# FrontierDevelopmentLab/2024-HL-SPI3S-SuNeRF

Hardware: AMD Instinct MI355X
Metric: ray-samples/sec (fwd+bwd, fused emission renderer) (higher is better)
Workload: dtype f32 (forward: every operand split into an fp16 head and an exact remainder, head products on the fp16 matrix cores + block-scaled fp8 products for the two cross terms; backward: fp16 MFMA, W^T as a single fp16 image (measured policy); fp32 accumulate and parameters)

## Files before the change

### 2024-hl-spi3s-sunerf_amd/csrc/bwd_pipe.hip

```cpp
#include "grad_common.h"
#include <mutex>
#include <vector>

namespace {

constexpr int PD = 256, PKS = PD / 16, PNT = PD / 32, PT = 8;
constexpr int WG = 512;
constexpr int WG_PRE = 256;
constexpr int NBUF = 4;
constexpr int NBUF_H = 5;
#ifndef PIPE_DMA_ON_WEIGHT
#define PIPE_DMA_ON_WEIGHT 2
#endif
#ifndef PIPE_ZD
#define PIPE_ZD 2
#endif
#ifndef PIPE_RING
#define PIPE_RING 16
#endif
#ifndef PIPE_POLL_LAG
#define PIPE_POLL_LAG 2
#endif
constexpr int RING = PIPE_RING;
constexpr int SLOT = PKS * 1024;
#ifndef PIPE_LDS_IMAGE
#define PIPE_LDS_IMAGE 1
#endif
static_assert(PIPE_LDS_IMAGE >= 0 && PIPE_LDS_IMAGE <= 2, "PIPE_LDS_IMAGE: 0, 1 or 2");
constexpr int FRAG_H = PIPE_LDS_IMAGE ? 1088 : 1024;
constexpr int BUF_HID = 24 * FRAG_H;
constexpr int BUF_IN = 16 * 1024;
constexpr int BUF_PRE = 19 * 1024;
constexpr unsigned SPIN_LIMIT = 50000000u;

constexpr unsigned ST_OK = 0, ST_START_TIMEOUT = 1, ST_PLACEMENT = 2, ST_WAIT_TIMEOUT = 3;

struct PipeArgs {
  const char* packedT;
  const char* act_stash;
  const char* dz_top;
  char* rings;
  unsigned* ctrl;
  float* partial;
  const float* g_raw;
  const unsigned* g_absmax_bits;
  float* partial_out;
  int64_t n_chunks_total;
  int S, n_chunks;
  int n_linear, d_out;
  int NP, NPX;
  int hi_only;
  int inject;
  unsigned* dbg;
};

__host__ __device__ inline size_t ctrl_counter_word(int n_links, int P, int link, int which) {
  return 64 + (((size_t)P * n_links + link) * 4 + which) * 32;
}
__host__ __device__ inline size_t ctrl_bytes(int NP, int n_links) { return (64 + (size_t)NP * n_links * 4 * 32) * 4; }

typedef __attribute__((address_space(1))) unsigned gu32;
__device__ __forceinline__ unsigned ld_agent(const unsigned* p) {
  return __hip_atomic_load((const gu32*)p, __ATOMIC_RELAXED, __HIP_MEMORY_SCOPE_AGENT);
}
__device__ __forceinline__ void st_agent(unsigned* p, unsigned v) {
  __hip_atomic_store((gu32*)p, v, __ATOMIC_RELAXED, __HIP_MEMORY_SCOPE_AGENT);
}

template <int POLICY>
__device__ __forceinline__ void dma_piece(const char* src_lane, unsigned lds_dst) {
  const unsigned d = __builtin_amdgcn_readfirstlane(lds_dst);
  if (POLICY == 1) asm volatile("s_mov_b32 m0, %1\n\ts_nop 0\n\tglobal_load_lds_dwordx4 %0, off nt" :: "v"(src_lane), "s"(d) : "memory");
  else if (POLICY == 2) asm volatile("s_mov_b32 m0, %1\n\ts_nop 0\n\tglobal_load_lds_dwordx4 %0, off sc1" :: "v"(src_lane), "s"(d) : "memory");
  else asm volatile("s_mov_b32 m0, %1\n\ts_nop 0\n\tglobal_load_lds_dwordx4 %0, off" :: "v"(src_lane), "s"(d) : "memory");
}
template <int POLICY>
__device__ __forceinline__ void dma_piece_s(const char* src_uniform, unsigned voff, unsigned lds_dst) {
  const unsigned d = __builtin_amdgcn_readfirstlane(lds_dst);
#ifndef PIPE_STREAM_BITS
#define PIPE_STREAM_BITS "nt"
#endif
  if (POLICY == 1) asm volatile("s_mov_b32 m0, %1\n\ts_nop 0\n\tglobal_load_lds_dwordx4 %0, %2 " PIPE_STREAM_BITS :: "v"(voff), "s"(d), "s"(src_uniform) : "memory");
  else if (POLICY == 2) asm volatile("s_mov_b32 m0, %1\n\ts_nop 0\n\tglobal_load_lds_dwordx4 %0, %2 sc1" :: "v"(voff), "s"(d), "s"(src_uniform) : "memory");
  else asm volatile("s_mov_b32 m0, %1\n\ts_nop 0\n\tglobal_load_lds_dwordx4 %0, %2" :: "v"(voff), "s"(d), "s"(src_uniform) : "memory");
}
__device__ __forceinline__ void dma_poll(const unsigned* src_lane, unsigned lds_dst) {
  const unsigned d = __builtin_amdgcn_readfirstlane(lds_dst);
  asm volatile("s_mov_b32 m0, %1\n\ts_nop 0\n\tglobal_load_lds_dword %0, off sc1" :: "v"(src_lane), "s"(d) : "memory");
}

__device__ __forceinline__ void store_tile(const f32x16& t, float* dst) {
  const Rsrc r = make_rsrc(dst, 16 * 64 * 4);
  const int lo4 = (int)(threadIdx.x & 63u) * 4;
#pragma unroll
  for (int g = 0; g < 16; ++g) {
    const float te = t[g];
    unsigned tv;
    asm volatile("v_accvgpr_read_b32 %0, %1" : "=v"(tv) : "a"(te));
    __builtin_amdgcn_raw_buffer_store_b32(tv, r, lo4, g * 256, 0);
    if ((g & 3) == 3) __builtin_amdgcn_sched_barrier(0);
  }
}

__device__ __forceinline__ void mfma_agpr(f32x16& acc, const half8& a, const half8& b) {
  asm volatile("v_mfma_f32_32x32x16_f16 %0, %1, %2, %0" : "+a"(acc) : "v"(a), "v"(b));
}
__device__ __forceinline__ void drain_matrix_pipe() { asm volatile("s_nop 15\n\ts_nop 15\n\ts_nop 15\n\ts_nop 15" ::: "memory"); }

#ifndef PIPE_KO_WREADS
#define PIPE_KO_WREADS 0
#endif
#if PIPE_KO_WREADS
#define TR_FIXED(R0, R1, R2, R3, OFF, var, base) asm volatile("" : "={v[" #R0 ":" #R3 "]}"(var) : "v"(base) : "memory")
#else
#define TR_FIXED(R0, R1, R2, R3, OFF, var, base)                                                                        \
  asm volatile("ds_read_b64_tr_b16 v[" #R0 ":" #R1 "], %1 offset:%2\n\tds_read_b64_tr_b16 v[" #R2 ":" #R3 "], %1 offset:%3" \
               : "={v[" #R0 ":" #R3 "]}"(var) : "v"(base), "i"(OFF), "i"((OFF) + 64) : "memory")
#endif
__device__ __forceinline__ unsigned tr_lane_offset_image(int lane) {
  if (PIPE_LDS_IMAGE == 0) return tr_lane_offset(lane);
  const int g = lane >> 4, i = lane & 15, q = i >> 2, p = i & 3;
  int row = (p >> 1) * 32 + 8 * (g >> 1) + q;
  if (PIPE_LDS_IMAGE == 2) row ^= 8 * (row >> 5);
  return (g & 1) * FRAG_H + row * 16 + (p & 1) * 8;
}
__device__ __forceinline__ unsigned frag_row_offset(int lane) { return (PIPE_LDS_IMAGE == 2 ? lane ^ (8 * (lane >> 5)) : lane) * 16; }

__device__ __forceinline__ void dz_tile(const f32x16& acc, const float* c0, const float* c1, half8& d0, half8& d1, float* bs) {
#pragma unroll
  for (int j = 0; j < 8; ++j) {
    const float p0 = acc[j] * c0[j], p1 = acc[8 + j] * c1[j];
    bs[j] += p0;
    bs[8 + j] += p1;
    d0[j] = (_Float16)sunerf_sat16(p0);
    d1[j] = (_Float16)sunerf_sat16(p1);
  }
}
#ifndef PIPE_TRIM
#define PIPE_TRIM 1
#endif
#ifndef PIPE_FP16_OVFL
#define PIPE_FP16_OVFL 1
#endif
#ifndef PIPE_DECODE_UNDER_CHAIN
#define PIPE_DECODE_UNDER_CHAIN 1
#endif
#if PIPE_DECODE_UNDER_CHAIN && !PIPE_TRIM
#error "PIPE_DECODE_UNDER_CHAIN is written on the register pairs of PIPE_TRIM"
#endif
typedef float v2f __attribute__((ext_vector_type(2)));
__device__ __forceinline__ void dz_tile_pairs(const f32x16& acc, const v2f* cs2, half8& d0, half8& d1, v2f* bs2) {
#pragma unroll
  for (int q = 0; q < 8; ++q) {
    const v2f a = {acc[2 * q], acc[2 * q + 1]};
    const v2f p = a * cs2[q];
    bs2[q] += p;
    const float x = PIPE_FP16_OVFL ? p.x : sunerf_sat16(p.x), y = PIPE_FP16_OVFL ? p.y : sunerf_sat16(p.y);
    if (q < 4) { d0[2 * q] = (_Float16)x; d0[2 * q + 1] = (_Float16)y; }
    else { d1[2 * q - 8] = (_Float16)x; d1[2 * q - 7] = (_Float16)y; }
  }
}
__device__ __forceinline__ half8 decode_phases_pairs(const v4u& p, v2f* cs2) {
  half8 h;
#pragma unroll
  for (int q = 0; q < 4; ++q) {
    v2f r = {(float)(p[q] & 0xffffu), (float)(p[q] >> 16)};
    r = r * (v2f){SUNERF_PHASE_SCALE, SUNERF_PHASE_SCALE};
    h[2 * q] = (_Float16)__builtin_amdgcn_sinf(r.x);
    h[2 * q + 1] = (_Float16)__builtin_amdgcn_sinf(r.y);
    cs2[q] = (v2f){__builtin_amdgcn_cosf(r.x), __builtin_amdgcn_cosf(r.y)};
  }
  return h;
}
__device__ __forceinline__ void decode_pair_first(unsigned w, v2f& r, v2f& c, float& s0) {
  r = (v2f){(float)(w & 0xffffu), (float)(w >> 16)};
  r = r * (v2f){SUNERF_PHASE_SCALE, SUNERF_PHASE_SCALE};
  s0 = __builtin_amdgcn_sinf(r.x);
  c.x = __builtin_amdgcn_cosf(r.x);
  asm volatile("" : "+v"(s0), "+v"(c.x), "+v"(r));
}
__device__ __forceinline__ void decode_pair_second(const v2f& r, v2f& c, float s0, half8& h, int q) {
  typedef _Float16 half2v __attribute__((ext_vector_type(2)));
  const float s1 = __builtin_amdgcn_sinf(r.y);
  c.y = __builtin_amdgcn_cosf(r.y);
  half2v pk = {(_Float16)s0, (_Float16)s1};
  asm volatile("" : "+v"(pk), "+v"(c.y));
  h[2 * q] = pk.x;
  h[2 * q + 1] = pk.y;
}
__device__ __forceinline__ void store_bias_sums(const float* bs, float* dst32) {
  const int lane = threadIdx.x & 63, h = lane >> 5;
#pragma unroll
  for (int g = 0; g < 16; ++g) {
    float v = bs[g];
#pragma unroll
    for (int d = 16; d >= 1; d >>= 1) v += __shfl_xor(v, d, 32);
    if ((lane & 31) == 0) dst32[16 * (g >> 3) + 8 * h + (g & 7)] = v;
  }
}

__device__ __forceinline__ void decode_phases(const v4u& p, float* sn, float* cs) {
#pragma unroll
  for (int e = 0; e < 8; ++e) {
    const unsigned w = p[e >> 1];
    const float rev = (float)((e & 1) ? (w >> 16) : (w & 0xffffu)) * SUNERF_PHASE_SCALE;
    sn[e] = __builtin_amdgcn_sinf(rev);
    cs[e] = __builtin_amdgcn_cosf(rev);
  }
}
__device__ __forceinline__ half8 to_half8(const float* v) {
  half8 r;
#pragma unroll
  for (int e = 0; e < 8; ++e) r[e] = (_Float16)v[e];
  return r;
}

typedef __attribute__((address_space(3))) unsigned lds_u32;
__device__ __forceinline__ unsigned lds_ld(unsigned addr) { return *(volatile lds_u32*)(uintptr_t)addr; }
__device__ __forceinline__ void lds_st(unsigned addr, unsigned v) { *(volatile lds_u32*)(uintptr_t)addr = v; }

__device__ __forceinline__ void barrier_mem() {
  asm volatile("s_waitcnt lgkmcnt(0)" ::: "memory");
  __builtin_amdgcn_s_barrier();
  asm volatile("" ::: "memory");
}

__device__ __forceinline__ bool spin_until(const unsigned* a0, const unsigned* a1, unsigned need, unsigned* status, unsigned& have, unsigned* stat) {
  const unsigned long long t0 = __builtin_amdgcn_s_memrealtime();
  stat[0] += 1;
  for (;;) {
    const unsigned v0 = ld_agent(a0), v1 = ld_agent(a1);
    have = v0 < v1 ? v0 : v1;
    if ((int)(have - need) >= 0) { stat[1] += (unsigned)(__builtin_amdgcn_s_memrealtime() - t0); return true; }
    if (ld_agent(status) != ST_OK) return false;
    if (__builtin_amdgcn_s_memrealtime() - t0 > SPIN_LIMIT) {
      st_agent(status, ST_WAIT_TIMEOUT);
      return false;
    }
    __builtin_amdgcn_s_sleep(8);
  }
}

template <bool HI_ONLY, bool TOP>
__device__ __forceinline__ void hidden_stage(const PipeArgs& a, char* smem, int P, int l, int j, int64_t cbeg, int n_my) {
  const int tid = threadIdx.x, lane = tid & 63;
  const int wave = __builtin_amdgcn_readfirstlane(tid >> 6);
  const int n_act = a.n_linear - 1, n_links = n_act - 1;
  const StashLayout SL(PD, a.n_linear, true);
  const unsigned lds0 = (unsigned)(uintptr_t)smem;
  const unsigned lds_dummy = lds0 + NBUF_H * BUF_HID;
  const unsigned lds_poll = lds_dummy + 1024;
  const unsigned lds_abort = lds_poll + NBUF_H * 256;
  unsigned* status = a.ctrl;
  const unsigned voff = frag_row_offset(lane);

  char* ring_in = TOP ? nullptr : a.rings + ((size_t)P * n_links + l) * RING * SLOT;
  char* ring_out = a.rings + ((size_t)P * n_links + (l - 1)) * RING * SLOT;
  const size_t act_chunk = SL.chunk_bytes();
  const char* srcP0 = a.act_stash + SL.h_off(l - 1) + (size_t)(8 * j) * 1024;
  const int64_t safe = cbeg < a.n_chunks_total ? cbeg : a.n_chunks_total - 1;

  constexpr int ZD = TOP ? NBUF_H - 1 : PIPE_ZD;
  const char *nz = nullptr, *np = nullptr;
  unsigned zdst = 0, pdst = 0;
  bool zreal = false, preal = false;
  const char* const safe_p = srcP0 + (size_t)safe * act_chunk;
  const char* const safe_z = TOP ? a.dz_top + (size_t)safe * SLOT : ring_in;
  const char* run_p = srcP0 + (size_t)cbeg * act_chunk;
  const char* run_z = TOP ? a.dz_top + (size_t)cbeg * SLOT : ring_in;
  int run_slot = 0, run_zbuf = 0, run_pbuf = 0;
  auto next_p = [&](int nxt) __attribute__((always_inline)) {
    preal = nxt < n_my;
    pdst = lds0 + run_pbuf * BUF_HID + 16 * FRAG_H;
    run_pbuf = run_pbuf + 1 == NBUF_H ? 0 : run_pbuf + 1;
    np = preal ? run_p : safe_p;
    run_p += act_chunk;
  };
  auto next_z = [&](int nxt) __attribute__((always_inline)) {
    if (nxt < 0) { zreal = false; nz = safe_z; return; }
    zreal = nxt < n_my;
    zdst = lds0 + run_zbuf * BUF_HID;
    run_zbuf = run_zbuf + 1 == NBUF_H ? 0 : run_zbuf + 1;
    nz = zreal ? run_z : safe_z;
    if (TOP) run_z += SLOT;
    else {
      run_slot = run_slot + 1 == RING ? 0 : run_slot + 1;
      run_z = run_slot == 0 ? ring_in : run_z + SLOT;
    }
  };
  auto piece_z = [&](int f) __attribute__((always_inline)) {
    const unsigned dst = zreal ? zdst + f * FRAG_H : lds_dummy;
    if (TOP) dma_piece_s<1>(nz + (size_t)f * 1024, voff, dst);
    else dma_piece_s<2>(nz + (size_t)f * 1024, voff, dst);
  };
  auto piece_p = [&](int f) __attribute__((always_inline)) { dma_piece_s<1>(np + (size_t)f * 1024, voff, preal ? pdst + f * FRAG_H : lds_dummy); };
  constexpr int NO = 2;
  constexpr int NP_D = PIPE_DMA_ON_WEIGHT == 0 ? 6 : PIPE_DMA_ON_WEIGHT == 1 ? 4 : 0;
  constexpr int NP_W = 6 - NP_D;
  constexpr int PER_D = NP_D + NO;
  auto min3 = [](int x, int y, int z) constexpr { return x < y ? (x < z ? x : z) : (y < z ? y : z); };
  constexpr int WAIT_LEFT = NP_D == 0 ? NO : min3((ZD - 1) * PER_D + (NP_D - 4) + NO, NP_D == 6 ? 2 * PER_D + NO : 63, 2 * PER_D);
  constexpr int DRAIN = (WAIT_LEFT + PER_D - 1) / PER_D + 1;
  auto w_wait = [min3](int per_w, bool gate_wave) constexpr {
    return min3(NP_W == 6 ? (ZD - 1) * per_w + 2 : 63, NP_W >= 2 ? 2 * per_w : 63, gate_wave ? PIPE_POLL_LAG * per_w - 2 : 63);
  };
  constexpr int W_WAIT_GATE = w_wait(NP_W + 2, true), W_WAIT_REST = w_wait(NP_W, false);

  static_assert(W_WAIT_GATE >= 0 && W_WAIT_GATE < 64 && WAIT_LEFT < 64, "vmcnt is a 6-bit counter");
  static_assert(ZD >= 1 && ZD <= NBUF_H - 1, "dZ fetch distance");

  if (wave < 4) {
#if defined(PIPE_PRIO) && PIPE_PRIO == 1
    __builtin_amdgcn_s_setprio(1);
#endif
#ifndef PIPE_PF
#define PIPE_PF 2
#endif
    constexpr int PF = PIPE_PF;
    const int U = 4 * j + wave;
    const int li = (a.n_linear - 2) - l;
    half8 wt_hi[PKS], wt_lo[HI_ONLY ? 1 : PKS];
    {
      const char* blk = a.packedT + (size_t)PNT * 1024 + ((size_t)li * PNT + U) * PKS * 2048 + lane * 16;
#pragma unroll
      for (int s = 0; s < PKS; ++s) {
        wt_hi[s] = *(const half8*)(blk + s * 2048);
        if constexpr (!HI_ONLY) wt_lo[s] = *(const half8*)(blk + s * 2048 + 1024);
      }
#pragma unroll
      for (int s = 0; s < PKS; ++s) {
        asm volatile("" : "+a"(wt_hi[s]));
        if constexpr (!HI_ONLY) asm volatile("" : "+a"(wt_lo[s]));
      }
    }
    char* scratch = a.rings + (size_t)a.NP * n_links * RING * SLOT + ((size_t)blockIdx.x * 4 + wave) * 2048;
    float cosn[16];
    v2f cosn2[8];
    typedef __attribute__((address_space(3))) v4u lds_v4u;
    typedef __attribute__((address_space(3))) half8 lds_half8;
    v4u dp[2];
    auto read_phases = [&](int b) __attribute__((always_inline)) {
      const unsigned at = lds0 + b * BUF_HID + (16 + 2 * wave) * FRAG_H + voff;
      dp[0] = *(const lds_v4u*)(uintptr_t)at;
      dp[1] = *(const lds_v4u*)(uintptr_t)(at + FRAG_H);
    };
    auto decode = [&](int b) __attribute__((always_inline)) {
      const unsigned at = lds0 + b * BUF_HID + (16 + 2 * wave) * FRAG_H + voff;
      if (PIPE_TRIM) {
        const half8 h0 = decode_phases_pairs(dp[0], cosn2), h1 = decode_phases_pairs(dp[1], cosn2 + 4);
        *(lds_half8*)(uintptr_t)at = h0;
        *(lds_half8*)(uintptr_t)(at + FRAG_H) = h1;
        return;
      }
      float sn[16];
      decode_phases(dp[0], sn, cosn);
      decode_phases(dp[1], sn + 8, cosn + 8);
      *(lds_half8*)(uintptr_t)at = to_half8(sn);
      *(lds_half8*)(uintptr_t)(at + FRAG_H) = to_half8(sn + 8);
    };
    bool stop = false;
    for (int it = -(NBUF_H - 1); it < 0; ++it) {
      asm volatile("s_waitcnt vmcnt(%0)" :: "i"(WAIT_LEFT) : "memory");
      barrier_mem();
      const unsigned ab = lds_ld(lds_abort + (it & 1) * 4);
      if (NP_D >= 4) next_z(it + ZD);
      if (NP_D == 6) next_p(it + NBUF_H - 1);
      const Rsrc sc = make_rsrc(scratch, 2048);
      const half8 zero = {0, 0, 0, 0, 0, 0, 0, 0};
      if (NP_D >= 4) { piece_z(wave); piece_z(4 + wave); piece_z(8 + wave); piece_z(12 + wave); }
      if (NP_D == 6) { piece_p(2 * wave); piece_p(2 * wave + 1); }
      buf_store(zero, sc, 0);
      buf_store(zero, sc, 1024);
      if (ab) { stop = true; break; }
      if (it == -1 && n_my > 0) { read_phases(0); decode(0); }
    }
    unsigned long long ph[6] = {0, 0, 0, 0, 0, 0};
    unsigned long long tl[5] = {0, 0, 0, 0, 0};
    const bool stamp = a.dbg != nullptr;
    char* out_z = ring_out;
    int out_slot = 0, buf = 0;
    float bs[16];
    v2f bs2[8];
#pragma unroll
    for (int g = 0; g < 16; ++g) bs[g] = 0.f;
#pragma unroll
    for (int q = 0; q < 8; ++q) bs2[q] = (v2f){0.f, 0.f};
    if (PIPE_FP16_OVFL) __builtin_amdgcn_s_setreg(1 | (23 << 6) | (0 << 11), 1);
    for (int it = 0; it < (stop ? 0 : n_my); ++it) {
      unsigned long long s0 = 0, s1 = 0, s2 = 0, s3 = 0;
      if (stamp) s0 = __builtin_amdgcn_s_memtime();
      asm volatile("s_waitcnt vmcnt(%0)" :: "i"(WAIT_LEFT) : "memory");
      const int nbuf = buf + 1 == NBUF_H ? 0 : buf + 1;
      const bool decode_next = it + 1 < n_my;
      if (stamp) s1 = __builtin_amdgcn_s_memtime();
      barrier_mem();
      if (stamp) s2 = __builtin_amdgcn_s_memtime();
      const unsigned ab = lds_ld(lds_abort + (it & 1) * 4);
      if (NP_D >= 4) next_z(it + ZD);
      if (NP_D == 6) next_p(it + NBUF_H - 1);
      const char* B = smem + (size_t)buf * BUF_HID;
      f32x16 dacc = {0};
      half8 bf[PF + 1];
      float cosc[16];
      v2f cosc2[8];
#pragma unroll
      for (int g = 0; g < 16; ++g) cosc[g] = cosn[g];
#pragma unroll
      for (int q = 0; q < 8; ++q) cosc2[q] = cosn2[q];
#if PIPE_DECODE_UNDER_CHAIN
      read_phases(nbuf);
      __builtin_amdgcn_sched_barrier(0);
      half8 hn[2];
      v2f dr = {0.f, 0.f};
      float ds0 = 0.f;
#endif
#pragma unroll
      for (int s = 0; s < PF; ++s) bf[s] = *(const half8*)(B + s * FRAG_H + voff);
#pragma unroll
      for (int ks = 0; ks < PKS; ++ks) {
        if (ks + PF < PKS) bf[(ks + PF) % (PF + 1)] = *(const half8*)(B + (ks + PF) * FRAG_H + voff);
        if constexpr (!HI_ONLY) dacc = __builtin_amdgcn_mfma_f32_32x32x16_f16(wt_lo[ks], bf[ks % (PF + 1)], dacc, 0, 0, 0);
        dacc = __builtin_amdgcn_mfma_f32_32x32x16_f16(wt_hi[ks], bf[ks % (PF + 1)], dacc, 0, 0, 0);
        if (NP_D >= 4) {
          if (ks == 0) piece_z(wave);
          if (ks == 2) piece_z(4 + wave);
          if (ks == 4) piece_z(8 + wave);
          if (ks == 6) piece_z(12 + wave);
        }
        if (NP_D == 6) {
          if (ks == 8) piece_p(2 * wave);
          if (ks == 10) piece_p(2 * wave + 1);
        }
#if PIPE_DECODE_UNDER_CHAIN
        __builtin_amdgcn_sched_barrier(0);
        if ((ks & 1) == 0) decode_pair_first(dp[ks >> 3][(ks >> 1) & 3], dr, cosn2[ks >> 1], ds0);
        else decode_pair_second(dr, cosn2[ks >> 1], ds0, hn[ks >> 3], (ks >> 1) & 3);
#else
        if (ks == 12 && decode_next) read_phases(nbuf);
#endif
        __builtin_amdgcn_sched_barrier(0);
      }
#if PIPE_DECODE_UNDER_CHAIN
      if (decode_next) {
        const unsigned at = lds0 + nbuf * BUF_HID + (16 + 2 * wave) * FRAG_H + voff;
        *(lds_half8*)(uintptr_t)at = hn[0];
        *(lds_half8*)(uintptr_t)(at + FRAG_H) = hn[1];
      }
#endif
      if (stamp) { asm volatile("" :: "v"(dacc)); s3 = __builtin_amdgcn_s_memtime(); }
      half8 d0, d1;
      const Rsrc ro = make_rsrc(out_z, SLOT);
      if (PIPE_TRIM) dz_tile_pairs(dacc, cosc2, d0, d1, bs2);
      else dz_tile(dacc, cosc, cosc + 8, d0, d1, bs);
      unsigned long long s3a = 0, s3b = 0;
      if (stamp) { asm volatile("" :: "v"(d0), "v"(d1)); s3a = __builtin_amdgcn_s_memtime(); }
      buf_store(d0, ro, (2 * U) * 1024);
      buf_store(d1, ro, (2 * U + 1) * 1024);
      if (stamp) s3b = __builtin_amdgcn_s_memtime();
      out_slot = out_slot + 1 == RING ? 0 : out_slot + 1;
      out_z = out_slot == 0 ? ring_out : out_z + SLOT;
      buf = nbuf;
#if !PIPE_DECODE_UNDER_CHAIN
      if (decode_next) decode(buf);
#endif
      if (stamp) {
        const unsigned long long s4 = __builtin_amdgcn_s_memtime();
        ph[0] += s1 - s0; ph[1] += s2 - s1; ph[2] += s3 - s2; ph[3] += s4 - s3; ph[4] += s3a - s3; ph[5] += s3b - s3;
        if (it == n_my / 2) { tl[0] = s0; tl[1] = s1; tl[2] = s2; tl[3] = s3; tl[4] = s4; }
      }
      if (ab) break;
    }
    asm volatile("s_waitcnt vmcnt(0)" ::: "memory");
    barrier_mem();
    if (PIPE_TRIM) {
#pragma unroll
      for (int q = 0; q < 8; ++q) { bs[2 * q] = bs2[q].x; bs[2 * q + 1] = bs2[q].y; }
    }
    store_bias_sums(bs, a.partial + ((size_t)(l - 1) * a.NP + P) * (PT * (PT + 1)) * 1024 + ((size_t)U * (PT + 1) + PT) * 1024);
    if (stamp && P == 0 && lane == 0) {
      unsigned long long* t = (unsigned long long*)(a.dbg + 256 * 8 * 4) + (((size_t)(blockIdx.x >> 3) * 8 + wave) * 8);
      for (int k = 0; k < 5; ++k) t[k] = tl[k];
    }
    if (stamp && wave == 1 && lane == 0) {
      unsigned* d = a.dbg + 256 * 8 + (size_t)blockIdx.x * 8;
      for (int k = 0; k < 6; ++k) d[k] = (unsigned)(ph[k] >> 4);
    }
    return;
  }

#if defined(PIPE_PRIO) && PIPE_PRIO == 2
  __builtin_amdgcn_s_setprio(1);
#endif
  const int v = wave - 4;
  const bool gatew = v == 0;
  const int rq = v >> 1, cq = v & 1;
  const int r0 = 4 * rq, c0 = 2 * cq;
  f32x16 acc[4][2];
  {
    half8 hz = {0, 0, 0, 0, 0, 0, 0, 0};
    asm volatile("s_nop 7" : "+v"(hz));
#pragma unroll
    for (int i = 0; i < 4; ++i) {
      asm volatile("v_mfma_f32_32x32x16_f16 %0, %1, %1, 0" : "=a"(acc[i][0]) : "v"(hz));
      asm volatile("v_mfma_f32_32x32x16_f16 %0, %1, %1, 0" : "=a"(acc[i][1]) : "v"(hz));
    }
  }
  unsigned* in_prod0 = a.ctrl + ctrl_counter_word(n_links, P, TOP ? 0 : l, 0);
  unsigned* in_prod1 = a.ctrl + ctrl_counter_word(n_links, P, TOP ? 0 : l, 1);
  unsigned* my_cons = a.ctrl + ctrl_counter_word(n_links, P, TOP ? 0 : l, 2 + j);
  unsigned* my_prod = a.ctrl + ctrl_counter_word(n_links, P, l - 1, j);
  unsigned* out_cons0 = a.ctrl + ctrl_counter_word(n_links, P, l - 1, 2 + (l == 1 ? j : 0));
  unsigned* out_cons1 = a.ctrl + ctrl_counter_word(n_links, P, l - 1, 2 + (l == 1 ? j : 1));
  const unsigned* poll_src = (lane & 3) == 0 ? in_prod0 : (lane & 3) == 1 ? in_prod1 : (lane & 3) == 2 ? out_cons0 : out_cons1;
  unsigned have_in = 0, have_out = 0;
  unsigned st_in[2] = {0, 0}, st_out[2] = {0, 0};
  const unsigned long long t_begin = __builtin_amdgcn_s_memrealtime();
  const unsigned laneoff = tr_lane_offset_image(lane);

  auto gate = [&](int itn) __attribute__((always_inline)) {
    const int nx = itn + ZD;
    const bool need_in = !TOP && nx >= 0 && nx < n_my && (int)(have_in - (unsigned)(nx + 1)) < 0;
    const bool need_out = itn >= RING && (int)(have_out - (unsigned)(itn - RING + 1)) < 0;
    if (need_in || need_out) {
      bool ok = true;
      if (lane == 0) {
        if (need_in) ok = spin_until(in_prod0, in_prod1, (unsigned)(nx + 1), status, have_in, st_in);
        if (ok && need_out) ok = spin_until(out_cons0, out_cons1, (unsigned)(itn - RING + 1), status, have_out, st_out);
        if (!ok) lds_st(lds_abort + (itn & 1) * 4, 1u);
      }
      have_in = __builtin_amdgcn_readfirstlane(have_in);
      have_out = __builtin_amdgcn_readfirstlane(have_out);
    }
  };
  if (gatew) {
    if (lane == 0) { lds_st(lds_abort, 0u); lds_st(lds_abort + 4, 0u); }
    gate(-(NBUF_H - 1));
  }

  bool aborted = false;
  unsigned long long tw = 0, tb = 0;
  unsigned long long t_wait = 0, t_bar = 0, tl[6] = {0, 0, 0, 0, 0, 0};
  const bool stamp = a.dbg != nullptr;
  int pslot = PIPE_POLL_LAG;
  auto top = [&](int it) __attribute__((always_inline)) {
    unsigned long long sa = 0, sb = 0;
    if (stamp) sa = __builtin_amdgcn_s_memtime();
    if (gatew) asm volatile("s_waitcnt vmcnt(%0)" :: "i"(W_WAIT_GATE) : "memory");
    else if (NP_W) asm volatile("s_waitcnt vmcnt(%0)" :: "i"(W_WAIT_REST) : "memory");
    if (stamp) sb = __builtin_amdgcn_s_memtime();
    barrier_mem();
    if (stamp) { t_wait = sb; t_bar = __builtin_amdgcn_s_memtime(); tw += sb - sa; tb += t_bar - sb; }
    const unsigned ab = lds_ld(lds_abort + (it & 1) * 4);
    if (gatew) {
      if (lane < 2) {
        const int pv = lane == 0 ? it + 1 : it - DRAIN + 1;
        st_agent(lane == 0 ? my_cons : my_prod, (unsigned)(pv > 0 ? pv : 0));
      }
      pslot = pslot + 1 == NBUF_H ? 0 : pslot + 1;
      dma_poll(poll_src, lds_poll + pslot * 256);
    }
    return ab;
  };
  auto w_piece = [&](int q) __attribute__((always_inline)) {
    if (q < 4) { if (NP_W == 6) piece_z(4 * q + v); }
    else if (NP_W >= 2) piece_p(2 * v + q - 4);
  };
  for (int it = -(NBUF_H - 1); it < 0; ++it) {
    const unsigned ab = top(it);
    if (NP_W == 6) next_z(it + ZD);
    if (NP_W >= 2) next_p(it + NBUF_H - 1);
#pragma unroll
    for (int q = 0; q < 6; ++q) w_piece(q);
    if (ab) { aborted = true; break; }
    if (gatew && it + 1 < n_my) gate(it + 1);
  }
  unsigned long long ph[4] = {0, 0, 0, 0};
  tw = 0; tb = 0;
  int buf = 0;
  for (int it = 0; it < (aborted ? 0 : n_my); ++it) {
    unsigned long long s0 = 0, s1 = 0, s2 = 0;
    if (stamp) s0 = __builtin_amdgcn_s_memtime();
    const unsigned ab = top(it);
    if (NP_W == 6) next_z(it + ZD);
    if (NP_W >= 2) next_p(it + NBUF_H - 1);
    if (stamp) s1 = __builtin_amdgcn_s_memtime();
    constexpr int PAIR = 2 * FRAG_H;
    const unsigned bufA = lds0 + buf * BUF_HID + laneoff + r0 * PAIR, bufB = lds0 + buf * BUF_HID + laneoff + 16 * FRAG_H + c0 * PAIR;
    half8 A0[4], B0[2], A1[4], B1[2];
    TR_FIXED(80, 81, 82, 83, 0 * PAIR, A0[0], bufA); TR_FIXED(84, 85, 86, 87, 1 * PAIR, A0[1], bufA);
    TR_FIXED(88, 89, 90, 91, 2 * PAIR, A0[2], bufA); TR_FIXED(92, 93, 94, 95, 3 * PAIR, A0[3], bufA);
    TR_FIXED(96, 97, 98, 99, 0 * PAIR, B0[0], bufB); TR_FIXED(100, 101, 102, 103, 1 * PAIR, B0[1], bufB);
    typedef __attribute__((address_space(3))) v4u lds_v4u;
    v4u pw = {0, 0, 0, 0};
    if (gatew) pw = *(const lds_v4u*)(uintptr_t)(lds_poll + buf * 256);
    asm volatile("s_waitcnt lgkmcnt(0)" ::: "memory");
    if (gatew) {
      asm volatile("" : "+v"(pw));
      const unsigned pi = pw[0] < pw[1] ? pw[0] : pw[1], qo = pw[2] < pw[3] ? pw[2] : pw[3];
      if ((int)(pi - have_in) > 0) have_in = pi;
      if ((int)(qo - have_out) > 0) have_out = qo;
      have_in = __builtin_amdgcn_readfirstlane(have_in);
      have_out = __builtin_amdgcn_readfirstlane(have_out);
      if (it + 1 < n_my) gate(it + 1);
    }
    if (stamp) s2 = __builtin_amdgcn_s_memtime();
    asm volatile("" : "+v"(A0[0]), "+v"(A0[1]), "+v"(A0[2]), "+v"(A0[3]), "+v"(B0[0]), "+v"(B0[1]));
    TR_FIXED(104, 105, 106, 107, 0 * PAIR + 256, A1[0], bufA); TR_FIXED(108, 109, 110, 111, 1 * PAIR + 256, A1[1], bufA);
    TR_FIXED(112, 113, 114, 115, 2 * PAIR + 256, A1[2], bufA); TR_FIXED(116, 117, 118, 119, 3 * PAIR + 256, A1[3], bufA);
    TR_FIXED(120, 121, 122, 123, 0 * PAIR + 256, B1[0], bufB); TR_FIXED(124, 125, 126, 127, 1 * PAIR + 256, B1[1], bufB);
#pragma unroll
    for (int ks = 0; ks < 2; ++ks) {
      if (ks == 1) {
        asm volatile("s_waitcnt lgkmcnt(0)" ::: "memory");
        asm volatile("" : "+v"(A1[0]), "+v"(A1[1]), "+v"(A1[2]), "+v"(A1[3]), "+v"(B1[0]), "+v"(B1[1]));
      }
      const half8 bf0 = ks ? B1[0] : B0[0], bf1 = ks ? B1[1] : B0[1];
      asm volatile("s_nop 1" ::: "memory");
#pragma unroll
      for (int i = 0; i < 4; ++i) {
        const half8 af = ks ? A1[i] : A0[i];
        mfma_agpr(acc[i][0], af, bf0);
        mfma_agpr(acc[i][1], af, bf1);
        if (4 * ks + i < NP_W) w_piece(6 - NP_W + 4 * ks + i);
        __builtin_amdgcn_sched_barrier(0);
// ... 255 lines not shown
    half8 dzo = {0, 0, 0, 0, 0, 0, 0, 0};
    float cs[2][16];
    if (it >= 0) {
#pragma unroll
      for (int f = 0; f < 4; ++f) {
        const unsigned at = lds0 + buf * BUF_PRE + (4 * wave + f) * 1024 + lane * 16;
        const v4u p = *(const lds_v4u*)(uintptr_t)at;
        float sn[8];
        decode_phases(p, sn, cs[f >> 1] + 8 * (f & 1));
        *(lds_half8*)(uintptr_t)at = to_half8(sn);
      }
      const int64_t chunk = cbeg + it;
      const int c = (int)(chunk % a.n_chunks);
      const int i = 32 * c + n;
      if (h == 0 && i < a.S) {
        const f32x2 g = *(const f32x2*)(smem + (size_t)buf * BUF_PRE + 18 * 1024 + n * 8);
        const float g0 = g[0] * gscale, g1 = a.d_out > 1 ? g[1] * gscale : 0.f;
        dzo[0] = (_Float16)g0;
        dzo[1] = (_Float16)g1;
        gsum0 += g0;
        gsum1 += g1;
      }
      if (wave == 0) *(half8*)(smem + (size_t)buf * BUF_PRE + 16 * 1024 + lane * 16) = dzo;
      else if (wave == 1) *(half8*)(smem + (size_t)buf * BUF_PRE + 17 * 1024 + lane * 16) = (half8){0, 0, 0, 0, 0, 0, 0, 0};
    }
    barrier_mem();
    issue_chunk(nxt, nxt & (NBUF - 1));
    if (it < 0) {
      const Rsrc sc = make_rsrc(scratch, 2048);
      const half8 zero = {0, 0, 0, 0, 0, 0, 0, 0};
#pragma unroll
      for (int k = 0; k < NO; ++k) buf_store(zero, sc, (k & 1) * 1024);
      continue;
    }
    const Rsrc ro = make_rsrc(a.dz_top + (size_t)(cbeg + it) * SLOT, SLOT);
#pragma unroll
    for (int t = 0; t < 2; ++t) {
      const int U = 2 * wave + t;
      f32x16 d = {0};
      d = __builtin_amdgcn_mfma_f32_32x32x16_f16(aT[t], dzo, d, 0, 0, 0);
      half8 d0, d1;
      dz_tile(d, cs[t], cs[t] + 8, d0, d1, bs[t]);
      buf_store(d0, ro, (2 * U) * 1024);
      buf_store(d1, ro, (2 * U + 1) * 1024);
    }
    const unsigned bufH = lds0 + buf * BUF_PRE + laneoff, bufA = bufH + 16 * 1024;
#pragma unroll
    for (int ks = 0; ks < 2; ++ks) {
      half4 alo, ahi, blo[2], bhi[2];
      tr_issue(bufA + ks * 256, alo, ahi);
#pragma unroll
      for (int t = 0; t < 2; ++t) tr_issue(bufH + (2 * (2 * wave + t)) * 1024 + ks * 256, blo[t], bhi[t]);
      asm volatile("s_waitcnt lgkmcnt(0)" ::: "memory");
      asm volatile("" : "+v"(alo), "+v"(ahi));
#pragma unroll
      for (int t = 0; t < 2; ++t) asm volatile("" : "+v"(blo[t]), "+v"(bhi[t]));
      const half8 af = join(alo, ahi);
#pragma unroll
      for (int t = 0; t < 2; ++t) acc[t] = __builtin_amdgcn_mfma_f32_32x32x16_f16(af, join(blo[t], bhi[t]), acc[t], 0, 0, 0);
    }
  }
  asm volatile("s_waitcnt vmcnt(0)" ::: "memory");
  float* out = a.partial_out + (size_t)blockIdx.x * (PT + 2) * 1024;
#pragma unroll
  for (int t = 0; t < 2; ++t) {
    store_tile(acc[t], out + (size_t)(2 * wave + t) * 1024);
    store_bias_sums(bs[t], out + (size_t)(PT + 1) * 1024 + (2 * wave + t) * 32);
  }
  if (wave == 0) {
#pragma unroll
    for (int d = 16; d >= 1; d >>= 1) { gsum0 += __shfl_xor(gsum0, d, 32); gsum1 += __shfl_xor(gsum1, d, 32); }
    if (lane < 32) out[(size_t)PT * 1024 + lane] = lane == 0 ? gsum0 : (lane == 1 ? gsum1 : 0.f);
  }
}

struct PipeLayout {
  int n_act, n_links, NPX, NP, grid;
  size_t sticky, dbg, ctrl, rings, dz_top, partial, partial_out, total;
  PipeLayout(int64_t n_chunks_total, int n_linear, int cus) {
    n_act = n_linear - 1;
    n_links = n_act - 1;
    grid = cus;
    NPX = (cus / 8) / (2 * n_act);
    NP = 8 * NPX;
    auto up = [](size_t v) { return (v + 255) / 256 * 256; };
    size_t off = 0;
    sticky = off; off += SUNERF_PIPE_WS_DEBUG;
    dbg = off; off += up((size_t)cus * 64 * sizeof(unsigned));
    ctrl = off; off += up(ctrl_bytes(NP, n_links));
    rings = off; off += up((size_t)NP * n_links * RING * SLOT + (size_t)cus * 4 * 2048);
    dz_top = off; off += up((size_t)(n_chunks_total > 0 ? n_chunks_total : 1) * SLOT);
    partial = off; off += up((size_t)n_act * NP * PT * (PT + 1) * 1024 * sizeof(float));
    partial_out = off; off += up((size_t)cus * (PT + 2) * 1024 * sizeof(float));
    total = off;
  }
};
static_assert(SUNERF_PIPE_WS_STICKY == 0 && SUNERF_PIPE_WS_DEBUG == 256, "fixed offsets of the workspace header");

struct TimedLaunch { hipEvent_t e0, e1; };
std::mutex g_timed_mutex;
std::vector<TimedLaunch> g_timed;

bool pipe_supported(int d_filter, int n_linear, int d_out, int cus) {
  return d_filter == PD && n_linear >= 3 && n_linear <= SUNERF_MAX_LAYERS && d_out >= 1 && d_out <= 2 && cus == 256 &&
         2 * (n_linear - 1) <= cus / 8;
}

int device_cus() {
  int dev = 0, cus = 0;
  (void)hipGetDevice(&dev);
  (void)hipDeviceGetAttribute(&cus, hipDeviceAttributeMultiprocessorCount, dev);
  return cus;
}

}

extern "C" size_t sunerf_bwd_pipe_workspace_bytes(int64_t n_rays, int n_samples, int d_filter, int n_linear) {
  const int cus = device_cus();
  if (n_rays < 0 || n_samples < 2 || !pipe_supported(d_filter, n_linear, 1, cus)) return 0;
  const int64_t n_chunks = (n_samples + 31) / 32;
  return PipeLayout(n_rays * n_chunks, n_linear, cus).total;
}

extern "C" int sunerf_mlp_backward_pipe(int d_filter, int n_linear, int d_out, const void* packedT, const void* act_stash,
                                        const float* g_raw, const void* g_absmax, int64_t n_rays, int n_samples,
                                        void* workspace, size_t workspace_bytes, float* const* grad_weights_host,
                                        float* const* grad_biases_host, int accumulate, int flags, void* stream) {
  if (!grad_weights_host || !grad_biases_host) return SUNERF_E_BADARG;
  if (n_rays <= 0 || n_samples < 2) return SUNERF_E_BADARG;
  if (!packedT || !act_stash || !g_raw || !g_absmax || !workspace) return SUNERF_E_BADARG;
  const int cus = device_cus();
  if (!pipe_supported(d_filter, n_linear, d_out, cus)) return SUNERF_E_UNSUPPORTED;
  hipStream_t st = (hipStream_t)stream;
  const int n_chunks = (n_samples + 31) / 32;
  const PipeLayout L(n_rays * n_chunks, n_linear, cus);
  if (workspace_bytes < L.total) return SUNERF_E_WORKSPACE;
  char* ws = (char*)workspace;
  PipeArgs a;
  a.packedT = (const char*)packedT; a.act_stash = (const char*)act_stash; a.dz_top = ws + L.dz_top; a.rings = ws + L.rings;
  a.ctrl = (unsigned*)(ws + L.ctrl); a.partial = (float*)(ws + L.partial); a.g_raw = g_raw;
  a.g_absmax_bits = (const unsigned*)g_absmax; a.partial_out = (float*)(ws + L.partial_out);
  a.n_chunks_total = n_rays * n_chunks; a.S = n_samples; a.n_chunks = n_chunks; a.n_linear = n_linear; a.d_out = d_out;
  a.NP = L.NP; a.NPX = L.NPX; a.hi_only = flags & 1; a.inject = (flags >> 8) & 1;
  a.dbg = (flags & 2) ? (unsigned*)(ws + L.dbg) : nullptr;
  hipError_t e;
  if ((e = hipMemsetAsync(ws + L.ctrl, 0, L.rings - L.ctrl, st)) != hipSuccess) return (int)e;
  const size_t lds_pre = (size_t)NBUF * BUF_PRE + 1024;
  constexpr size_t lds_pipe = (size_t)NBUF_H * BUF_HID + 1024 + NBUF_H * 256 + 64;
  static_assert(lds_pipe <= 160 * 1024 && (size_t)NBUF * BUF_IN + 1024 + NBUF * 256 + 64 <= lds_pipe, "LDS of a CU: 160 KiB");
  if ((e = hipFuncSetAttribute((const void*)bwd_prologue_kernel, hipFuncAttributeMaxDynamicSharedMemorySize, (int)lds_pre)) != hipSuccess) return (int)e;
  if ((e = hipFuncSetAttribute((const void*)bwd_pipe_kernel<false>, hipFuncAttributeMaxDynamicSharedMemorySize, (int)lds_pipe)) != hipSuccess) return (int)e;
  if ((e = hipFuncSetAttribute((const void*)bwd_pipe_kernel<true>, hipFuncAttributeMaxDynamicSharedMemorySize, (int)lds_pipe)) != hipSuccess) return (int)e;
  TimedLaunch tl = {nullptr, nullptr};
  if (flags & 0x80) {
    if ((e = hipEventCreate(&tl.e0)) != hipSuccess) return (int)e;
    if ((e = hipEventCreate(&tl.e1)) != hipSuccess) { (void)hipEventDestroy(tl.e0); return (int)e; }
  }
  SUNERF_CLEAR_ERROR();
  hipLaunchKernelGGL(bwd_prologue_kernel, dim3((unsigned)cus), dim3(WG_PRE), lds_pre, st, a);
  SUNERF_CHECK_LAUNCH();
  if (tl.e0) (void)hipEventRecord(tl.e0, st);
  if (a.hi_only) hipLaunchKernelGGL(bwd_pipe_kernel<true>, dim3((unsigned)cus), dim3(WG), lds_pipe, st, a);
  else hipLaunchKernelGGL(bwd_pipe_kernel<false>, dim3((unsigned)cus), dim3(WG), lds_pipe, st, a);
  if (tl.e0) {
    (void)hipEventRecord(tl.e1, st);
    std::lock_guard<std::mutex> lock(g_timed_mutex);
    g_timed.push_back(tl);
  }
  SUNERF_CHECK_LAUNCH();
  ReduceArgs r;
  const size_t slot = (size_t)PT * (PT + 1) * 1024;
  for (int i = 0; i < n_linear; ++i) {
    if (!grad_weights_host[i] || !grad_biases_host[i]) return SUNERF_E_BADARG;
    r.gW[i] = grad_weights_host[i];
    r.gb[i] = grad_biases_host[i];
    if (i < n_linear - 1) {
      r.partial[i] = a.partial + (size_t)i * L.NP * slot;
      r.split[i] = L.NP;
      r.slot[i] = slot;
    } else {
      r.partial[i] = a.partial_out;
      r.split[i] = cus;
      r.slot[i] = (size_t)(PT + 2) * 1024;
    }
    if (i < n_linear - 2) {
      r.bias[i] = r.partial[i] + (size_t)PT * 1024;
      r.bias_split[i] = L.NP;
      r.bias_slot[i] = slot;
      r.bias_tr[i] = (size_t)(PT + 1) * 1024;
    } else {
      r.bias[i] = a.partial_out + (size_t)(i == n_linear - 1 ? PT : PT + 1) * 1024;
      r.bias_split[i] = cus;
      r.bias_slot[i] = (size_t)(PT + 2) * 1024;
      r.bias_tr[i] = 32;
    }
  }
  r.g_absmax_bits = (const unsigned*)g_absmax; r.n_linear = n_linear; r.D = d_filter; r.d_out = d_out; r.accumulate = accumulate;
  r.sumsq = (const float*)((const char*)packedT + sunerf_packed_mlp_t_bytes(d_filter, n_linear) - SUNERF_MAX_LAYERS * sizeof(float));
  r.status = a.ctrl;
  r.sticky = (unsigned*)(ws + L.sticky);
  hipLaunchKernelGGL(reduce_grads_kernel, dim3(PT * (PT + 1) * 1024 / 256, n_linear), dim3(256), 0, st, r);
  SUNERF_CHECK_LAUNCH();
  return 0;
}

extern "C" int sunerf_bwd_pipe_kernel_time(double* total_ms, int* launches) {
  std::vector<TimedLaunch> mine;
  {
    std::lock_guard<std::mutex> lock(g_timed_mutex);
    mine.swap(g_timed);
  }
  double sum = 0.0;
  int n = 0, rc = 0;
  for (const TimedLaunch& t : mine) {
    float ms = 0.f;
    hipError_t e = hipEventSynchronize(t.e1);
    if (e == hipSuccess) e = hipEventElapsedTime(&ms, t.e0, t.e1);
    if (e == hipSuccess) { sum += ms; ++n; } else rc = (int)e;
    (void)hipEventDestroy(t.e0);
    (void)hipEventDestroy(t.e1);
  }
  if (total_ms) *total_ms = sum;
  if (launches) *launches = n;
  return rc;
}
```

Before: 210.4 million.

## Accumulate dH chain in VGPRs and ping-pong cosine buffers across unrolled chunks

The backward dH MFMA chain now takes the weights from AGPRs and accumulates in VGPRs, starting with a zero-accumulator MFMA, and a short fixed nop wait replaces the implicit accumulator readback. The cosine buffers for the current and next chunk swap roles by unrolling the loop two chunks at a time, which removes the per-iteration copy of the cosines, and the B-fragment prefetch distance grows to 3. The intent is to cut register moves and copy overhead on the critical MFMA-to-epilogue path. The risks are higher VGPR pressure, a hand-chosen nop count that may not cover the MFMA latency, and a larger unrolled body. It also adds event cleanup on launch errors.

```diff
diff --git a/2024-hl-spi3s-sunerf_amd/csrc/bwd_pipe.hip b/2024-hl-spi3s-sunerf_amd/csrc/bwd_pipe.hip
--- a/2024-hl-spi3s-sunerf_amd/csrc/bwd_pipe.hip
+++ b/2024-hl-spi3s-sunerf_amd/csrc/bwd_pipe.hip
@@ -105,6 +105,11 @@
 __device__ __forceinline__ void mfma_agpr(f32x16& acc, const half8& a, const half8& b) {
   asm volatile("v_mfma_f32_32x32x16_f16 %0, %1, %2, %0" : "+a"(acc) : "v"(a), "v"(b));
 }
+__device__ __forceinline__ void mfma_dh_vgpr(f32x16& acc, const half8& a, const half8& b, bool first) {
+  if (first) asm volatile("v_mfma_f32_32x32x16_f16 %0, %1, %2, 0" : "=&v"(acc) : "a"(a), "v"(b));
+  else asm volatile("v_mfma_f32_32x32x16_f16 %0, %1, %2, %0" : "+v"(acc) : "a"(a), "v"(b));
+}
+__device__ __forceinline__ void dh_tile_ready(f32x16& acc) { asm volatile("s_nop 15\n\ts_nop 3" : "+v"(acc)); }
 __device__ __forceinline__ void drain_matrix_pipe() { asm volatile("s_nop 15\n\ts_nop 15\n\ts_nop 15\n\ts_nop 15" ::: "memory"); }
 
 #ifndef PIPE_KO_WREADS
@@ -147,6 +152,15 @@
 #endif
 #if PIPE_DECODE_UNDER_CHAIN && !PIPE_TRIM
 #error "PIPE_DECODE_UNDER_CHAIN is written on the register pairs of PIPE_TRIM"
+#endif
+#ifndef PIPE_COS_SWAP
+#define PIPE_COS_SWAP 1
+#endif
+#ifndef PIPE_DH_VGPR
+#define PIPE_DH_VGPR 1
+#endif
+#if PIPE_COS_SWAP && !PIPE_DECODE_UNDER_CHAIN
+#error "PIPE_COS_SWAP is written on the decoder of PIPE_DECODE_UNDER_CHAIN"
 #endif
 typedef float v2f __attribute__((ext_vector_type(2)));
 __device__ __forceinline__ void dz_tile_pairs(const f32x16& acc, const v2f* cs2, half8& d0, half8& d1, v2f* bs2) {
@@ -174,7 +188,14 @@
 }
 __device__ __forceinline__ void decode_pair_first(unsigned w, v2f& r, v2f& c, float& s0) {
   r = (v2f){(float)(w & 0xffffu), (float)(w >> 16)};
+#if PIPE_DH_VGPR
+  float rx = r.x * SUNERF_PHASE_SCALE;
+  asm volatile("" : "+v"(rx));
+  const float ry = r.y * SUNERF_PHASE_SCALE;
+  r = (v2f){rx, ry};
+#else
   r = r * (v2f){SUNERF_PHASE_SCALE, SUNERF_PHASE_SCALE};
+#endif
   s0 = __builtin_amdgcn_sinf(r.x);
   c.x = __builtin_amdgcn_cosf(r.x);
   asm volatile("" : "+v"(s0), "+v"(c.x), "+v"(r));
@@ -314,7 +335,7 @@
     __builtin_amdgcn_s_setprio(1);
 #endif
 #ifndef PIPE_PF
-#define PIPE_PF 2
+#define PIPE_PF (PIPE_DH_VGPR ? 3 : 2)
 #endif
     constexpr int PF = PIPE_PF;
     const int U = 4 * j + wave;
@@ -386,7 +407,12 @@
 #pragma unroll
     for (int q = 0; q < 8; ++q) bs2[q] = (v2f){0.f, 0.f};
     if (PIPE_FP16_OVFL) __builtin_amdgcn_s_setreg(1 | (23 << 6) | (0 << 11), 1);
+#if PIPE_COS_SWAP
+    v2f cosm2[8];
+    auto chunk = [&](const int it, const v2f* cr2, v2f* cw2) __attribute__((always_inline)) -> bool {
+#else
     for (int it = 0; it < (stop ? 0 : n_my); ++it) {
+#endif
       unsigned long long s0 = 0, s1 = 0, s2 = 0, s3 = 0;
       if (stamp) s0 = __builtin_amdgcn_s_memtime();
       asm volatile("s_waitcnt vmcnt(%0)" :: "i"(WAIT_LEFT) : "memory");
@@ -399,14 +425,22 @@
       if (NP_D >= 4) next_z(it + ZD);
       if (NP_D == 6) next_p(it + NBUF_H - 1);
       const char* B = smem + (size_t)buf * BUF_HID;
+#if PIPE_DH_VGPR
+      f32x16 dacc;
+#else
       f32x16 dacc = {0};
+#endif
       half8 bf[PF + 1];
       float cosc[16];
       v2f cosc2[8];
+#if !PIPE_COS_SWAP
 #pragma unroll
       for (int g = 0; g < 16; ++g) cosc[g] = cosn[g];
 #pragma unroll
       for (int q = 0; q < 8; ++q) cosc2[q] = cosn2[q];
+      const v2f* cr2 = cosc2;
+      v2f* cw2 = cosn2;
+#endif
 #if PIPE_DECODE_UNDER_CHAIN
       read_phases(nbuf);
       __builtin_amdgcn_sched_barrier(0);
@@ -419,8 +453,13 @@
 #pragma unroll
       for (int ks = 0; ks < PKS; ++ks) {
         if (ks + PF < PKS) bf[(ks + PF) % (PF + 1)] = *(const half8*)(B + (ks + PF) * FRAG_H + voff);
+#if PIPE_DH_VGPR
+        if constexpr (!HI_ONLY) mfma_dh_vgpr(dacc, wt_lo[ks], bf[ks % (PF + 1)], ks == 0);
+        mfma_dh_vgpr(dacc, wt_hi[ks], bf[ks % (PF + 1)], HI_ONLY && ks == 0);
+#else
         if constexpr (!HI_ONLY) dacc = __builtin_amdgcn_mfma_f32_32x32x16_f16(wt_lo[ks], bf[ks % (PF + 1)], dacc, 0, 0, 0);
         dacc = __builtin_amdgcn_mfma_f32_32x32x16_f16(wt_hi[ks], bf[ks % (PF + 1)], dacc, 0, 0, 0);
+#endif
         if (NP_D >= 4) {
           if (ks == 0) piece_z(wave);
           if (ks == 2) piece_z(4 + wave);
@@ -433,8 +472,8 @@
         }
 #if PIPE_DECODE_UNDER_CHAIN
         __builtin_amdgcn_sched_barrier(0);
-        if ((ks & 1) == 0) decode_pair_first(dp[ks >> 3][(ks >> 1) & 3], dr, cosn2[ks >> 1], ds0);
-        else decode_pair_second(dr, cosn2[ks >> 1], ds0, hn[ks >> 3], (ks >> 1) & 3);
+        if ((ks & 1) == 0) decode_pair_first(dp[ks >> 3][(ks >> 1) & 3], dr, cw2[ks >> 1], ds0);
+        else decode_pair_second(dr, cw2[ks >> 1], ds0, hn[ks >> 3], (ks >> 1) & 3);
 #else
         if (ks == 12 && decode_next) read_phases(nbuf);
 #endif
@@ -447,10 +486,15 @@
         *(lds_half8*)(uintptr_t)(at + FRAG_H) = hn[1];
       }
 #endif
+#if PIPE_DH_VGPR
+      dh_tile_ready(dacc);
+#elif PIPE_COS_SWAP
+      asm volatile("" : "+a"(dacc));
+#endif
       if (stamp) { asm volatile("" :: "v"(dacc)); s3 = __builtin_amdgcn_s_memtime(); }
       half8 d0, d1;
       const Rsrc ro = make_rsrc(out_z, SLOT);
-      if (PIPE_TRIM) dz_tile_pairs(dacc, cosc2, d0, d1, bs2);
+      if (PIPE_TRIM) dz_tile_pairs(dacc, cr2, d0, d1, bs2);
       else dz_tile(dacc, cosc, cosc + 8, d0, d1, bs);
       unsigned long long s3a = 0, s3b = 0;
       if (stamp) { asm volatile("" :: "v"(d0), "v"(d1)); s3a = __builtin_amdgcn_s_memtime(); }
@@ -468,8 +512,19 @@
         ph[0] += s1 - s0; ph[1] += s2 - s1; ph[2] += s3 - s2; ph[3] += s4 - s3; ph[4] += s3a - s3; ph[5] += s3b - s3;
         if (it == n_my / 2) { tl[0] = s0; tl[1] = s1; tl[2] = s2; tl[3] = s3; tl[4] = s4; }
       }
+#if !PIPE_COS_SWAP
       if (ab) break;
     }
+#else
+      return ab != 0;
+    };
+    {
+      bool quit = stop;
+      int it = 0;
+      for (; !quit && it + 1 < n_my; it += 2) quit = chunk(it, cosn2, cosm2) || chunk(it + 1, cosm2, cosn2);
+      if (!quit && it < n_my) chunk(it, cosn2, cosm2);
+    }
+#endif
     asm volatile("s_waitcnt vmcnt(0)" ::: "memory");
     barrier_mem();
     if (PIPE_TRIM) {
@@ -1031,22 +1086,27 @@
   if ((e = hipFuncSetAttribute((const void*)bwd_pipe_kernel<false>, hipFuncAttributeMaxDynamicSharedMemorySize, (int)lds_pipe)) != hipSuccess) return (int)e;
   if ((e = hipFuncSetAttribute((const void*)bwd_pipe_kernel<true>, hipFuncAttributeMaxDynamicSharedMemorySize, (int)lds_pipe)) != hipSuccess) return (int)e;
   TimedLaunch tl = {nullptr, nullptr};
+  auto drop_events = [&tl]() {
+    if (tl.e0) (void)hipEventDestroy(tl.e0);
+    if (tl.e1) (void)hipEventDestroy(tl.e1);
+    tl.e0 = tl.e1 = nullptr;
+  };
   if (flags & 0x80) {
-    if ((e = hipEventCreate(&tl.e0)) != hipSuccess) return (int)e;
-    if ((e = hipEventCreate(&tl.e1)) != hipSuccess) { (void)hipEventDestroy(tl.e0); return (int)e; }
+    if ((e = hipEventCreate(&tl.e0)) != hipSuccess) { tl.e0 = nullptr; return (int)e; }
+    if ((e = hipEventCreate(&tl.e1)) != hipSuccess) { tl.e1 = nullptr; drop_events(); return (int)e; }
   }
   SUNERF_CLEAR_ERROR();
   hipLaunchKernelGGL(bwd_prologue_kernel, dim3((unsigned)cus), dim3(WG_PRE), lds_pre, st, a);
-  SUNERF_CHECK_LAUNCH();
+  if ((e = hipGetLastError()) != hipSuccess) { drop_events(); return (int)e; }
   if (tl.e0) (void)hipEventRecord(tl.e0, st);
   if (a.hi_only) hipLaunchKernelGGL(bwd_pipe_kernel<true>, dim3((unsigned)cus), dim3(WG), lds_pipe, st, a);
   else hipLaunchKernelGGL(bwd_pipe_kernel<false>, dim3((unsigned)cus), dim3(WG), lds_pipe, st, a);
+  if ((e = hipGetLastError()) != hipSuccess) { drop_events(); return (int)e; }
   if (tl.e0) {
     (void)hipEventRecord(tl.e1, st);
     std::lock_guard<std::mutex> lock(g_timed_mutex);
     g_timed.push_back(tl);
   }
-  SUNERF_CHECK_LAUNCH();
   ReduceArgs r;
   const size_t slot = (size_t)PT * (PT + 1) * 1024;
   for (int i = 0; i < n_linear; ++i) {
```

Result: no change. 212.3 million, median of 6 (+0.9%).
